# mattreturn1/ComputerVision_ObjectDetection_FeatureMatching

Measured on AMD Instinct MI355X. Metric: matches+homographies/sec (10k x 10k SIFT, 50k RANSAC iters) at 1/2/4/8 GPUs, higher is better.
Workload: dtype i8-MFMA exact-int distances (i32 acc), fp64 DLT/Jacobi, fp32 reprojection; 1 GPU; c4: one global batch of 256 scenes x 1 model set, 10000x10000 descriptors, maxIters 50000, scenes sharded over 1 GPU(s) (256 on rank 0); problems_per_gpu=256, global_batch=256, parallelism=dp1, batches_in_flight=16, dist_backend=nccl, hw_queues=24

## Files before the change

computervision_objectdetection_featurematching_amd/csrc/mim_internal.h:

```cpp
#pragma once
#include <hip/hip_runtime.h>
#include <stdint.h>

#include "knn_schedule.h"
#include "knn_topk_merge.h"

namespace mim {

constexpr int kDim = 128;
constexpr int kTileRows = 64;
constexpr int kTileBytes = kTileRows * kDim;
constexpr int kNormWords = 4 * kTileRows;
constexpr int kWave = 64;
#ifndef MIM_KNN_STAGE
#define MIM_KNN_STAGE 4
#endif
constexpr int kKnnStage = MIM_KNN_STAGE;

struct SetDev {
    const int8_t* frag;
    const int* norm;
    const float* f32;
    const float2* kp;
    int n;
    int n_tiles;
    int* flags;
};

struct PrepJob {
    const float* src;
    int8_t* frag;
    int* norm;
    int* flags;
    int n;
    int tile0;
};

struct Top2 {
    float k1; int i1; float k2; int i2;
};

struct ProbDev {
    SetDev q, t;
    int nsplit;
    int q_pad;
    long long part_off;
    long long good_off;
    long long it_off;
};


struct HamWork {
    const uint32_t* q;
    const uint32_t* t;
    Top2* out;
    int nq;
    int q0;
    int r0, r1;
    int wdw;
    int pad_;
};

struct HamCrossWork {
    HamWork w;
    uint32_t* colmin;
};

struct CrossDev {
    const uint32_t* colmin;
    int shadow;
    int pad_;
};


struct FltWork {
    const float* q;
    const float* t;
    Top2* out;
    int nq;
    int q0;
    int r0, r1;
    int dim;
    int dp;
};


struct TopkHamWork {
    const uint32_t* q;
    const uint32_t* t;
    TopkEnt* out;
    int nq;
    int q0;
    int r0, r1;
    int wdw;
    int pad_;
};

struct TopkFltWork {
    const float* q;
    const float* t;
    TopkEnt* out;
    int nq;
    int q0;
    int r0, r1;
    int dim;
    int dp;
    int nt;
    int vec;
};

struct TopkProb {
    const TopkEnt* parts;
    int32_t* idx;
    float* dist;
    int nq;
    int nsplit;
    int q_pad;
    int pad_;
};

struct RansacState {
    long long stream_pos;
    int produced;
    int fail_iter;
    int fail_run;
    int niters;
    int max_good;
    int best_iter;
    int next_iter;
    int done;
    int n;
    int active;
    int lo_max;
    unsigned long long modM;
    float sa, sb;
    float smax;
    int defer;
};

struct RansacParams {
    double thresh;
    double conf;
    int max_iters;
    float ratio;
    int min_good, min_inliers;
    double det_lo, det_hi;
    int cand_cap;
    int rep_cap;
};

}

namespace mim {
constexpr int kCandPerProblem = 1024;
constexpr int kIrrBlock = 16384;
constexpr int kRansacDefSlots = 16;
#ifndef MIM_CHECK_PER
#define MIM_CHECK_PER 4
#endif
constexpr int kRansacDefRoundAttempts = 256 * MIM_CHECK_PER;
constexpr int kIrrCap = 4096;

struct SamplerClass {
    long long base;
    int leader;
    int cwlen;
    int delta;
    int wlen;
    int pad_[2];
};
struct SamplerClassSlot {
    unsigned long long key;
    int end;
    int pad_;
};

struct RansacBufs {
    RansacState* state;
    int4* samples;
    float* hyp;
    int* counts;
    int2* bounds;
    double* best_h;
    int* cand;
    int* ncand;
    int* cex;
    double* cH;
    int* decided;
    uint8_t* flags;
    uint8_t* irr_bits;
    long long flag_cap;
    int* irr;
    int* irr_cnt;
    uint32_t* pass_bits;
    void* chains;
    int2* defer;
    int* defer_n;
    int def_rounds;
    int irr_blocks;
    SamplerClass* cls;
    SamplerClassSlot* cls_tab;
    int cls_tab_n;
    const uint32_t* stream;
    long long stream_len;
    float4* inl;
    uint4* tiles;
    int* err;
    hipStream_t s2;
    hipEvent_t ev_fork;
    hipEvent_t ev_samp[2];
};
}

#include <string>
#include <vector>
#include "../../include/mim.h"
namespace mim {
struct SiftWs;
SiftWs* sift_ws_create();
void sift_ws_destroy(SiftWs* w);
int sift_detect_compute(SiftWs* w, hipStream_t st, const uint8_t* img, int rows, int cols, long long step,
                        const uint8_t* mask, long long mstep, int max_kp, mim_keypoint* kps, float* desc, int* n_out,
                        std::string& err);
int sift_detect_compute_scales(std::vector<SiftWs*>& ws, hipStream_t st, const uint8_t* img, int rows, int cols,
                               long long step, int n_scales, const float* scales, int max_kp, mim_keypoint* kps,
                               float* desc, int* n_out, std::string& err);
int sift_resize_u8(SiftWs* w, hipStream_t st, const uint8_t* src, int rows, int cols, long long step, uint8_t* dst,
                   int drows, int dcols, double fx, double fy, std::string& err);
struct SiftDevOut {
    const mim_keypoint* kp;
    const float* desc;
    int n;
};
int sift_scales_device(std::vector<SiftWs*>& ws, hipStream_t st, const uint8_t* img, int rows, int cols,
                       long long step, int channels, int n_scales, const float* scales, SiftDevOut* out,
                       std::string& err);
int sift_bgr2gray_u8(SiftWs* w, hipStream_t st, const uint8_t* bgr, int rows, int cols, long long step, uint8_t* gray,
                     std::string& err);
int sift_copy_sets(const SiftDevOut* out, int n, float* const* ddesc, float2* const* dkp, hipStream_t st);
int sift_debug_pyramid(SiftWs* w, hipStream_t st, int* n_oct, int* orows, int* ocols, float* planes, long long cap,
                       long long* need, int* counters, std::string& err);
}
```

computervision_objectdetection_featurematching_amd/csrc/ransac.hip:

```cpp
#include <float.h>

#include <algorithm>
#include <climits>
#include <cstdio>
#include <cstdlib>
#include <vector>

#include "../../include/mim.h"
#include "mim_debug.h"
#include "mim_internal.h"

namespace mim {

__device__ __forceinline__ double d_hypot(double a, double b) {
    a = fabs(a);
    b = fabs(b);
    const bool ab = a > b;
    const double big = ab ? a : b, sm = ab ? b : a;
    const double r = sm / big;
    const double res = big * sqrt(1 + r * r);
    return (ab || b > 0) ? res : 0.0;
}

template <int n> __device__ __forceinline__ int pk(int i, int j) {
    static_assert(n <= 16, "packed index masks");
    return (int)(((unsigned)(i & 15) * (unsigned)((2 * n - 1 - i) & 31)) >> 1) + (j - i - 1);
}

template <int n> __device__ __forceinline__ int pk_any(int a, int b) {
    const int i = min(a, b), j = max(a, b);
    return pk<n>(i, j);
}

template <int n, int S>
__device__ void jacobi_fast(double* __restrict__ A, double* __restrict__ W, double* __restrict__ V,
                            double (&Ws)[n], int (&perm)[n]) {
#define AU(i, j) A[pk<n>((i), (j)) * S]
    const int trash = n * (n - 1) / 2 + n + n * n;
    const double eps = DBL_EPSILON;
#pragma unroll
    for (int i = 0; i < n; i++)
#pragma unroll
        for (int j = 0; j < n; j++) V[(i * n + j) * S] = i == j ? 1.0 : 0.0;
    int indR[n], indC[n];
#pragma unroll
    for (int k = 0; k < n; k++) {
        indR[k] = 0;
        indC[k] = 0;
        if (k < n - 1) {
            int m = k + 1;
            double mv = fabs(AU(k, k + 1));
#pragma unroll
            for (int i = k + 2; i < n; i++) {
                const double val = fabs(AU(k, i));
                if (mv < val) mv = val, m = i;
            }
            indR[k] = m;
        }
        if (k > 0) {
            int m = 0;
            double mv = fabs(AU(0, k));
#pragma unroll
            for (int i = 1; i < k; i++) {
                const double val = fabs(AU(i, k));
                if (mv < val) mv = val, m = i;
            }
            indC[k] = m;
        }
    }
    for (int iters = 0; iters < n * n * 30; iters++) {
        double vr[n], vc[n];
#pragma unroll
        for (int i = 0; i < n - 1; i++) vr[i] = A[(pk<n>(i, i + 1) + indR[i] - i - 1) * S];
#pragma unroll
        for (int i = 1; i < n; i++) vc[i] = A[pk_any<n>(indC[i], i) * S];
        int k = 0, l = indR[0];
        double mv = fabs(vr[0]), p = vr[0];
#pragma unroll
        for (int i = 1; i < n - 1; i++) {
            const double val = fabs(vr[i]);
            const bool u = mv < val;
            mv = u ? val : mv;
            k = u ? i : k;
            l = u ? indR[i] : l;
            p = u ? vr[i] : p;
        }
#pragma unroll
        for (int i = 1; i < n; i++) {
            const double val = fabs(vc[i]);
            const bool u = mv < val;
            mv = u ? val : mv;
            k = u ? indC[i] : k;
            l = u ? i : l;
            p = u ? vc[i] : p;
        }
        if (fabs(p) <= eps) break;
        const double wk = W[k * S], wl = W[l * S];
        double a0[n], b0[n], vk[n], vl[n];
#pragma unroll
        for (int i = 0; i < n; i++) {
            const bool vi = i != k && i != l;
            a0[i] = A[(vi ? pk_any<n>(i, k) : 0) * S];
            b0[i] = A[(vi ? pk_any<n>(i, l) : 0) * S];
            vk[i] = V[(k * n + i) * S];
            vl[i] = V[(l * n + i) * S];
        }
        const double y = (wl - wk) * 0.5;
        double t = fabs(y) + d_hypot(p, y);
        const double q = fabs(p) / t;
        double s = t * sqrt(1 + q * q);
        const double c = t / s;
        s = p / s;
        t = copysign(q, p) * p;
        s = y < 0 ? -s : s;
        t = y < 0 ? -t : t;
        AU(k, l) = 0;
        W[k * S] = wk - t;
        W[l * S] = wl + t;
        double rk[n], rl[n];
#pragma unroll
        for (int i = 0; i < n; i++) {
            const bool vi = i != k && i != l;
            const double na = a0[i] * c - b0[i] * s;
            const double nb = a0[i] * s + b0[i] * c;
            A[(vi ? pk_any<n>(i, k) : trash) * S] = na;
            A[(vi ? pk_any<n>(i, l) : trash) * S] = nb;
            rk[i] = vi ? na : 0.0;
            rl[i] = vi ? nb : 0.0;
            V[(k * n + i) * S] = vk[i] * c - vl[i] * s;
            V[(l * n + i) * S] = vk[i] * s + vl[i] * c;
        }
        int rkR = -1, rkC = -1, rlR = -1, rlC = -1;
        double bkR = 0, bkC = 0, blR = 0, blC = 0;
#pragma unroll
        for (int m = 0; m < n; m++) {
            const double ak = fabs(rk[m]), al = fabs(rl[m]);
            const bool u1 = m > k && (rkR < 0 || bkR < ak);
            const bool u2 = m < k && (rkC < 0 || bkC < ak);
            const bool u3 = m > l && (rlR < 0 || blR < al);
            const bool u4 = m < l && (rlC < 0 || blC < al);
            bkR = u1 ? ak : bkR; rkR = u1 ? m : rkR;
            bkC = u2 ? ak : bkC; rkC = u2 ? m : rkC;
            blR = u3 ? al : blR; rlR = u3 ? m : rlR;
            blC = u4 ? al : blC; rlC = u4 ? m : rlC;
        }
#pragma unroll
        for (int i = 0; i < n; i++) {
            indR[i] = (i == k && i < n - 1) ? rkR : ((i == l && i < n - 1) ? rlR : indR[i]);
            indC[i] = (i == k && i > 0) ? rkC : ((i == l && i > 0) ? rlC : indC[i]);
        }
    }
#pragma unroll
    for (int i = 0; i < n; i++) {
        Ws[i] = W[i * S];
        perm[i] = i;
    }
#pragma unroll
    for (int k = 0; k < n - 1; k++) {
// ... 953 lines not shown
        if (w < wave) r = max(r, wred[w]);
        all = max(all, wred[w]);
    }
    return r;
}

__device__ __forceinline__ int block_min(int v, int* wred) {
    const int lane = threadIdx.x & 63, wave = threadIdx.x >> 6, nw = blockDim.x >> 6;
    v = wave_min(v);
    __syncthreads();
    if (lane == 0) wred[wave] = v;
    __syncthreads();
    int r = INT_MAX;
    for (int w = 0; w < nw; ++w) r = min(r, wred[w]);
    return r;
}

__global__ __launch_bounds__(kWalkThreads) void ransac_walk_kernel(const RansacState* __restrict__ st,
                                                                    const uint8_t* __restrict__ flags, int wcap,
                                                                    int c1, const int* __restrict__ irr,
                                                                    const int* __restrict__ irr_cnt, int irr_blocks,
                                                                    ChainSegs* __restrict__ chains,
                                                                    const SamplerClass* __restrict__ cls) {
    __shared__ ChainWalkShared sh;
    const int p = blockIdx.x, tid = threadIdx.x, lane = tid & 63;
    const SamplerClass C = cls[p];
    ChainSegs* G = chains + p;
    if (C.leader < 0) {
        if (tid == 0) G->T = -1;
        return;
    }
    const int wlen = C.delta + C.wlen;
    const int pl = C.leader;
    const uint8_t* F = flags + (long long)pl * wcap;
    const int nb = min((wlen + kIrrBlock - 1) / kIrrBlock, kIrrBlocksMax);
    {
        const int cnt = tid < nb ? irr_cnt[(long long)pl * irr_blocks + tid] : 0;
        const int bad = tid < nb && cnt < 0 ? tid : INT_MAX;
        int total;
        const int off = block_excl_sum(max(cnt, 0), sh.wred, total);
        const int cut = min(block_min(bad, sh.wred2), nb);
        if (tid <= nb) sh.boff[tid] = tid < nb ? off : 0;
        __syncthreads();
        if (tid == 0) {
            sh.cut = cut;
            sh.n_entries = cut > 0 ? sh.boff[cut - 1] + irr_cnt[(long long)pl * irr_blocks + cut - 1] : 0;
            sh.limit = min(wlen, cut * kIrrBlock);
            sh.stop = 0;
        }
        __syncthreads();
    }
    int s = C.delta, nwalk = 0, limit = sh.limit;
    const int E = sh.n_entries, cut = sh.cut;
    for (int eb = 0; eb < E; eb += kChainEntries) {
        const int ee = min(E, eb + kChainEntries);
        for (int e = eb + tid; e < ee; e += kWalkThreads) {
            int lo = 0, hi = cut - 1;
            while (lo < hi) {
                const int mid = (lo + hi + 1) >> 1;
                if (sh.boff[mid] <= e) lo = mid; else hi = mid - 1;
            }
            const int q = irr[((long long)pl * irr_blocks + lo) * kIrrCap + (e - sh.boff[lo])];
            sh.q[e - eb] = q;
            sh.f[e - eb] = F[q];
        }
        __syncthreads();
        if (tid < 64) {
            bool stop = false;
            for (int e0 = eb; e0 < ee && !stop; e0 += 64) {
                const int e = e0 + lane;
                const int q = e < ee ? sh.q[e - eb] : INT_MAX;
                const int f = e < ee ? (int)sh.f[e - eb] : 0;
                for (;;) {
                    const unsigned long long m = __ballot(q >= s && q < limit && ((q - s) & 3) == 0);
                    if (!m) break;
                    const int k = uni(__builtin_ctzll(m));
                    const int qq = __builtin_amdgcn_readlane(q, k), ff = __builtin_amdgcn_readlane(f, k);
                    if (ff == kAttemptSerial || nwalk == kChainSegs) {
                        limit = qq;
                        stop = true;
                        break;
                    }
                    if (lane == 0) {
                        G->seg_s[nwalk] = s;
                        G->seg_q[nwalk] = qq;
                        G->seg_f[nwalk] = (uint8_t)ff;
                    }
                    ++nwalk;
                    s = uni(qq + 4 + ((ff & 0x7F) >> 1));
                }
            }
            if (lane == 0 && stop) sh.stop = 1;
        }
        __syncthreads();
        if (sh.stop) break;
    }
    if (tid < 64) {
        if (lane == 0) {
            const int tail = s < limit ? (limit - s + 3) >> 2 : 0;
            G->seg_s[nwalk] = s;
            sh.nseg = nwalk;
            sh.tail = tail;
            G->nseg = nwalk;
            G->tail = tail;
            G->s_end = s + 4 * tail;
            G->wbase = C.base;
            G->wlen = wlen;
        }
    }
    __syncthreads();
    const int nseg = sh.nseg;
    int v[kWalkSegsPer], sum = 0;
#pragma unroll
    for (int k = 0; k < kWalkSegsPer; ++k) {
        const int j = kWalkSegsPer * tid + k;
        v[k] = j < nseg ? ((G->seg_q[j] - G->seg_s[j]) >> 2) + 1 : (j == nseg ? sh.tail : 0);
        sum += v[k];
    }
    int total;
    int base = block_excl_sum(sum, sh.wred, total);
#pragma unroll
    for (int k = 0; k < kWalkSegsPer; ++k) {
        const int j = kWalkSegsPer * tid + k;
        if (j <= nseg + 1) G->A[j] = base;
        if (j <= nseg)
            for (int b = (base + kCheckBlock - 1) / kCheckBlock; b * kCheckBlock < base + v[k] && b < kChainBlk; ++b)
                G->blk_seg[b] = j;
        base += v[k];
    }
    if (tid == 0) G->T = total;
}

__device__ __forceinline__ int chain_pos(const ChainSegs* G, int j, int t, bool& irregular) {
    irregular = j < G->nseg && t == G->A[j + 1] - 1;
    return irregular ? G->seg_q[j] : G->seg_s[j] + 4 * (t - G->A[j]);
}

__device__ __forceinline__ int chain_seg(const ChainSegs* G, int t) {
    int lo = 0, hi = G->nseg;
    while (lo < hi) {
        const int mid = (lo + hi + 1) >> 1;
        if (G->A[mid] <= t) lo = mid; else hi = mid - 1;
    }
    return lo;
}


constexpr int kCheckPer = MIM_CHECK_PER;
constexpr int kCheckSegs = 8;
#ifndef MIM_PROBE_CHECK
#define MIM_PROBE_CHECK 0
#endif
constexpr int kDefSlots = kRansacDefSlots;
#ifndef MIM_CHECK_LDS
#define MIM_CHECK_LDS 0
#endif
constexpr int kCheckLdsPts = MIM_CHECK_LDS ? 2048 : 1;
static_assert(kCheckBlock * kCheckPer == kRansacDefRoundAttempts, "check round size shared with api.cpp");

__device__ __attribute__((noinline)) bool check_deferred(int qe, const uint32_t* __restrict__ stream, long long slen,
                                                         unsigned N, unsigned long long modM,
                                                         const float4* __restrict__ P) {
    const long long qq = qe < 0 ? -(long long)qe - 1 : qe;
    int ix[4];
    if (qe < 0) {
        resolve_at(qq, stream, slen, N, modM, ix);
    } else {
#pragma unroll
        for (int k = 0; k < 4; ++k) ix[k] = (int)fastmod(stream[qq + k], modM, N);
    }
    const float4 a = P[ix[0]], bp = P[ix[1]], c = P[ix[2]], d = P[ix[3]];
    const float s4[8] = {a.x, a.y, bp.x, bp.y, c.x, c.y, d.x, d.y};
    const float t4[8] = {a.z, a.w, bp.z, bp.w, c.z, c.w, d.z, d.w};
    return check_subset(s4, t4);
}

#ifndef MIM_CHECK_OCC
#define MIM_CHECK_OCC 1
#endif
__global__ __launch_bounds__(kCheckBlock, MIM_CHECK_OCC) void ransac_check_kernel(const ChainSegs* __restrict__ chains,
                                                                   const ProbDev* __restrict__ probs,
                                                                   const float4* __restrict__ pts,
                                                                   const RansacState* __restrict__ st,
                                                                   const uint32_t* __restrict__ stream, long long slen,
                                                                   uint32_t* __restrict__ pass_bits, int wcap, int bpp,
                                                                   int2* __restrict__ defer, int* __restrict__ defer_n,
                                                                   int def_rounds, int n_probs) {
    __shared__ uint32_t words[kCheckBlock * kCheckPer / 32];
    __shared__ int def_t[kCheckBlock * kCheckPer], def_q[kCheckBlock * kCheckPer];
    __shared__ int4 seg_tab[kCheckSegs];
    __shared__ int n_def;
    __shared__ float4 spts[kCheckLdsPts];
    const int x = blockIdx.x & 7, jx = blockIdx.x >> 3, np8 = (n_probs + 7) >> 3;
    const int p = x + 8 * (jx % np8), kb0 = jx / np8, lane = threadIdx.x & 63;
    if (p >= n_probs) return;
    const ChainSegs* G = chains + p;
    const int T = G->T;
    if (T <= 0) return;
    const RansacState S = st[p];
    const float4* P = pts + probs[p].good_off;
    const bool lds = MIM_CHECK_LDS && S.n <= kCheckLdsPts;
    if (lds) {
        for (int i = threadIdx.x; i < S.n; i += kCheckBlock) spts[i] = P[i];
    }
    for (int b = kb0; b * kCheckBlock * kCheckPer < T; b += bpp) {
    const int base = b * kCheckBlock * kCheckPer;
    const int nseg = G->nseg;
    const int bb = base / kCheckBlock;
    const int j0 = bb < kChainBlk ? G->blk_seg[bb] : chain_seg(G, base);
    if (threadIdx.x < kCheckSegs) {
        const int j = j0 + threadIdx.x;
        seg_tab[threadIdx.x] = make_int4(G->A[min(j, nseg + 1)], G->A[min(j + 1, nseg + 1)], G->seg_s[min(j, nseg)],
                                         G->seg_q[min(j, max(nseg - 1, 0))]);
    }
    int segA[kCheckSegs];
#pragma unroll
    for (int k = 1; k < kCheckSegs; ++k) segA[k] = j0 + k <= nseg ? G->A[j0 + k] : INT_MAX;
    const unsigned N = (unsigned)S.n;
    if (threadIdx.x == 0) n_def = 0;
    __syncthreads();
    int q[kCheckPer];
    bool irr[kCheckPer], valid[kCheckPer];
#pragma unroll
    for (int r = 0; r < kCheckPer; ++r) {
        const int t = base + r * kCheckBlock + threadIdx.x;
        valid[r] = t < T;
        int k = 0;
#pragma unroll
        for (int i = 1; i < kCheckSegs; ++i) k += t >= segA[i];
        const int4 e = seg_tab[k];
        int j = j0 + k, pos;
        bool irregular;
        if (j < nseg && t >= e.y) {
            while (j < nseg && t >= G->A[j + 1]) ++j;
            pos = chain_pos(G, j, t, irregular);
        } else {
            irregular = j < nseg && t == e.y - 1;
            pos = irregular ? e.w : e.z + 4 * (t - e.x);
        }
        q[r] = valid[r] ? (int)(G->wbase + pos) : 0;
        irr[r] = valid[r] && irregular;
    }
    typedef unsigned uint4a4 __attribute__((ext_vector_type(4), aligned(4)));
    unsigned raw[kCheckPer][4];
#pragma unroll
    for (int r = 0; r < kCheckPer; ++r) {
        const uint4a4 v = *reinterpret_cast<const uint4a4*>(stream + q[r]);
        raw[r][0] = v.x; raw[r][1] = v.y; raw[r][2] = v.z; raw[r][3] = v.w;
    }
    int idx[kCheckPer][4];
#pragma unroll
    for (int r = 0; r < kCheckPer; ++r)
#pragma unroll
        for (int k = 0; k < 4; ++k) idx[r][k] = valid[r] ? (int)fastmod(raw[r][k], S.modM, N) : 0;
    float4 g[kCheckPer][4];
    __syncthreads();
    if (lds) {
#pragma unroll
        for (int r = 0; r < kCheckPer; ++r)
#pragma unroll
            for (int k = 0; k < 4; ++k) g[r][k] = spts[idx[r][k]];
    } else {
#pragma unroll
        for (int r = 0; r < kCheckPer; ++r)
#pragma unroll
            for (int k = 0; k < 4; ++k) g[r][k] = P[idx[r][k]];
    }
    const bool listed = b < def_rounds;
#pragma unroll
    for (int r = 0; r < kCheckPer; ++r) {
        const float s4[8] = {g[r][0].x, g[r][0].y, g[r][1].x, g[r][1].y, g[r][2].x, g[r][2].y, g[r][3].x, g[r][3].y};
        const float t4[8] = {g[r][0].z, g[r][0].w, g[r][1].z, g[r][1].w, g[r][2].z, g[r][2].w, g[r][3].z, g[r][3].w};
        bool clear = true;
        const bool pass32 = MIM_PROBE_CHECK == 3 ? (s4[0] + s4[1] + s4[2] + s4[3] + s4[4] + s4[5] + s4[6] + s4[7] +
                                                    t4[0] + t4[1] + t4[2] + t4[3] + t4[4] + t4[5] + t4[6] + t4[7]) > 4000.f
                          : MIM_PROBE_CHECK == 2 ? s4[0] != t4[1] : check_subset_fp32(s4, t4, clear);
        MIM_DEBUG_CHECK(!valid[r] || !clear || pass32 == check_subset(s4, t4),
                        "[check] fp32 checkSubset %d differs from fp64 (p=%d t=%d)\n", (int)pass32, p,
                        base + r * kCheckBlock + (int)threadIdx.x);
        const bool defer = MIM_PROBE_CHECK == 0 && valid[r] && (irr[r] || !clear);
        const unsigned long long m = __ballot(valid[r] && !defer && pass32);
        const int wl = (r * kCheckBlock + (threadIdx.x & ~63)) >> 5;
        if (lane == 0) words[wl] = (uint32_t)m;
        if (lane == 32) words[wl + 1] = (uint32_t)(m >> 32);
        if (defer) {
            const int slot = atomicAdd(&n_def, 1);
            def_t[slot] = r * kCheckBlock + threadIdx.x;
            def_q[slot] = irr[r] ? -q[r] - 1 : q[r];
        }
    }
    __syncthreads();
    MIM_DEBUG_PRINT(threadIdx.x == 0 && (p == 0 || p == 100), "[check] p=%d b=%d bpp=%d T=%d nseg=%d n_def=%d wlen=%d\n",
                    p, b, bpp, T, nseg, n_def, G->wlen);
    const int nl = listed ? min(n_def, kDefSlots) : 0;
    if (listed && threadIdx.x == 0) defer_n[(long long)p * def_rounds + b] = nl;
    if (threadIdx.x < nl)
        defer[((long long)p * def_rounds + b) * kDefSlots + threadIdx.x] =
            make_int2(base + def_t[threadIdx.x], def_q[threadIdx.x]);
    if (n_def > nl) {
        for (int e = nl + threadIdx.x; e < n_def; e += kCheckBlock) {
            const int tl = def_t[e];
            if (check_deferred(def_q[e], stream, slen, N, S.modM, P)) atomicOr(&words[tl >> 5], 1u << (tl & 31));
        }
        __syncthreads();
    }
    uint32_t* PB = pass_bits + (long long)p * (wcap / 32);
    if (threadIdx.x < kCheckBlock * kCheckPer / 32 && (base + 32 * (int)threadIdx.x) < T)
        PB[(base >> 5) + threadIdx.x] = words[threadIdx.x];
    __syncthreads();
    }
}

__global__ __launch_bounds__(256) void ransac_check_defer_kernel(const ChainSegs* __restrict__ chains,
                                                                 const ProbDev* __restrict__ probs,
                                                                 const float4* __restrict__ pts,
                                                                 const RansacState* __restrict__ st,
                                                                 const uint32_t* __restrict__ stream, long long slen,
                                                                 uint32_t* __restrict__ pass_bits, int wcap,
                                                                 const int2* __restrict__ defer,
                                                                 const int* __restrict__ defer_n, int def_rounds,
                                                                 int nblk, int n_probs) {
    const int p = blockIdx.x / nblk;
    const int j = (blockIdx.x % nblk) * 256 + threadIdx.x, round = j / kDefSlots, e = j % kDefSlots;
    if (p >= n_probs || round >= def_rounds) return;
    const int T = chains[p].T;
    if (round * (kCheckBlock * kCheckPer) >= T) return;
    const long long rr = (long long)p * def_rounds + round;
    if (e >= defer_n[rr]) return;
    const int2 en = defer[rr * kDefSlots + e];
    const int t = en.x, qe = en.y;
    if (check_deferred(qe, stream, slen, (unsigned)st[p].n, st[p].modM, pts + probs[p].good_off))
        atomicOr(pass_bits + (long long)p * (wcap / 32) + (t >> 5), 1u << (t & 31));
}

template <class Fn>
__device__ __forceinline__ void pass_visit(const uint32_t* __restrict__ PB, int t0, int t1, Fn&& fn) {
    if (t0 >= t1) return;
    const int wl = (t1 - 1) >> 5;
    for (int w0 = t0 >> 5; w0 <= wl; w0 += 8) {
        uint32_t wd[8];
#pragma unroll
        for (int k = 0; k < 8; ++k) wd[k] = PB[min(w0 + k, wl)];
#pragma unroll
        for (int k = 0; k < 8; ++k) {
            const int w = w0 + k;
            if (w > wl) break;
            const int lo_b = max(t0 - 32 * w, 0), hi_b = min(t1 - 32 * w, 32);
            const uint32_t rm = (hi_b == 32 ? 0xFFFFFFFFu : ((1u << hi_b) - 1)) & ~((1u << lo_b) - 1);
            uint32_t bits = wd[k] & rm;
            while (bits) {
                const int bit = __builtin_ctz(bits);
                bits &= bits - 1;
                fn(32 * w + bit);
            }
        }
    }
}

struct ChainCountShared {
    int wred[kChainThreads / 64];
    int wred2[kChainThreads / 64];
    int t_need;
};

__global__ __launch_bounds__(kChainThreads) void ransac_count_kernel(RansacState* __restrict__ st,
                                                                     const ProbDev* __restrict__ probs,
                                                                     const ChainSegs* __restrict__ chains,
                                                                     const uint32_t* __restrict__ pass_bits,
                                                                     const uint8_t* __restrict__ flags, int wcap,
                                                                     int4* __restrict__ samples, int c1,
                                                                     const SamplerClass* __restrict__ cls) {
    __shared__ ChainCountShared sh;
    const int p = blockIdx.x, tid = threadIdx.x;
    const ChainSegs* G = chains + p;
    const int T = G->T;
    if (T < 0) return;
    RansacState S = st[p];
    const int target = min(c1, S.niters);
    if (S.produced >= target) return;
    const long long wbase = G->wbase;
    const uint32_t* PB = pass_bits + (long long)p * (wcap / 32);
    const int words = (T + 31) >> 5;
    const int wpt = (words + kChainThreads - 1) / kChainThreads;
    const int t0 = min(T, tid * wpt * 32), t1 = min(T, t0 + wpt * 32);
    int cnt = 0, first = -1, last = -1;
    pass_visit(PB, t0, t1, [&](int t) {
        if (first < 0) first = t;
        last = t;
        ++cnt;
    });
    int total;
    const int base = block_excl_sum(cnt, sh.wred, total);
    const int v0 = -1 - S.fail_run;
    int last_all;
    const int prev = block_excl_max(cnt ? last : INT_MIN, v0, sh.wred2, last_all);
    int ev = (cnt && first - prev - 1 >= 10000) ? prev + 10000 : kNoEvent;
    if (tid == 0 && T - 1 - last_all >= 10000) ev = min(ev, last_all + 10000);
    const int t_fail = block_min(ev, sh.wred);
    const int need = target - S.produced;
    if (tid == 0) sh.t_need = kNoEvent;
    __syncthreads();
    if (base < need && need <= base + cnt) {
        int k = need - base;
        pass_visit(PB, t0, t1, [&](int t) {
            if (--k == 0) sh.t_need = t;
        });
    }
    __syncthreads();
    const int t_need = sh.t_need;
    int keep;
    if (t_fail < t_need) {
        int before = 0;
        if (cnt && last < t_fail) before = cnt;
        else if (cnt && first < t_fail) pass_visit(PB, t0, t1, [&](int t) { before += t < t_fail; });
        int tot_before;
        block_excl_sum(before, sh.wred, tot_before);
        keep = tot_before;
    } else {
        keep = t_need != kNoEvent ? need : total;
    }
    if (base < keep) {
        int4* out = samples + probs[p].it_off + S.produced;
        int r = base, j = -1, a_next = 0, a_j = 0, s_j = 0, q_j = 0;
        pass_visit(PB, t0, t1, [&](int t) {
            if (r < keep) {
                if (j < 0 || t >= a_next) {
                    j = j < 0 ? chain_seg(G, t) : j + 1;
                    while (j < G->nseg && t >= G->A[j + 1]) ++j;
                    a_j = G->A[j];
                    a_next = G->A[j + 1];
                    s_j = G->seg_s[j];
                    q_j = j < G->nseg ? G->seg_q[j] : 0;
                }
                const bool irregular = j < G->nseg && t == a_next - 1;
                const int pos = irregular ? q_j : s_j + 4 * (t - a_j);
                out[r] = make_int4((int)(wbase + pos), irregular ? -2 : -1, 0, 0);
            }
            ++r;
        });
    }
    if (tid == 0) {
        if (t_fail < t_need) {
            S.produced += keep;
            S.fail_iter = S.produced;
            S.fail_run = 10000;
        } else if (t_need != kNoEvent) {
            const int j = chain_seg(G, t_need);
            bool irregular;
            const int pos = chain_pos(G, j, t_need, irregular);
            const int len = irregular ? 4 + ((flags[(long long)cls[p].leader * wcap + pos] & 0x7F) >> 1) : 4;
            S.produced = target;
            S.stream_pos = wbase + pos + len;
            S.fail_run = 0;
        } else {
            S.produced += total;
            S.fail_run = total > 0 ? T - 1 - last_all : S.fail_run + T;
            S.stream_pos = wbase + G->s_end;
        }
        store_sampler_state(st + p, S);
    }
}


// ... 1872 lines not shown
                            for (int j = 0; j < 8; ++j) s += sh.A[8 * i + j] * sh.d[j];
                            temp_d[i] = -s + 2 * sh.v[i];
                        }
                        double dS = 0;
                        for (int i = 0; i < 8; ++i) dS += sh.d[i] * temp_d[i];
                        const double R = (Scur - Sd) / (fabs(dS) > DBL_EPSILON ? dS : 1);
                        if (R > Rhi) {
                            lambda *= 0.5;
                            if (lambda < lc) lambda = 0;
                        } else if (R < Rlo) {
                            double t = 0;
                            for (int i = 0; i < 8; ++i) t += sh.d[i] * sh.v[i];
                            double nu = (Sd - Scur) / (fabs(t) > DBL_EPSILON ? t : 1) + 2;
                            nu = fmin(fmax(nu, 2.), 10.);
                            if (lambda == 0) {
                                const double maxval = inv_diag_max8(ew, eperm, sh.J9 + 36);
                                lambda = lc = 1. / maxval;
                                nu *= 0.5;
                            }
                            lambda *= nu;
                        }
                        if (tid == 0) {
                            sh.lambda = lambda;
                            sh.lc = lc;
                            sh.accept = Sd < Scur;
                            if (sh.accept) {
                                sh.S = Sd;
                                for (int i = 0; i < 8; ++i) sh.x[i] = sh.xd[i];
                            }
                        }
                    }
                    wsync();
                    if (sh.accept) {
#if MIM_LM_MERGE
                        rinf = rinf_d;
#else
                        for (int i = 0; i < 8; ++i) x[i] = sh.x[i];
                        lm_normal(X, k, x, sh.lm, sh.nrm, rinf);
#endif
                        if (tid == 0) {
                            int e = 0;
                            for (int a = 0; a < 8; ++a)
                                for (int b = a; b < 8; ++b, ++e) sh.A[a * 8 + b] = sh.A[b * 8 + a] = sh.nrm[e];
                            for (int i = 0; i < 8; ++i) sh.v[i] = sh.nrm[36 + i];
                            sh.rinf = rinf;
                        }
                    }
                    MIM_RT_MARK(t_norm);
                    ++iter;
                    if (tid == 0) sh.proceed = iter < 10 && sh.dinf >= FLT_EPSILON && sh.rinf >= FLT_EPSILON;
                    wsync();
                    const bool proceed = sh.proceed;
                    wsync();
                    if (!proceed) break;
                }
#if MIM_REFINE_TIMING
                rt_iters = iter;
#endif
                if (tid < 8) sh.H[tid] = sh.x[tid];
                wsync();
            } else if (tid == 0) {
                for (int i = 0; i < 9; ++i) sh.H[i] = sh.Hb[i];
            }
            wsync();
        } else {
            for (int i = tid; i < ng; i += 64) mask[i] = 0;
            if (tid == 0) sh.n_inl = 0;
        }
    }
    wsync();
    if (tid != 0) return;
#if MIM_REFINE_TIMING
    {
        const unsigned long long tot = wall_clock64() - rt_start;
        if (tot > 20000)
            printf("[refine-timing] p=%d ng=%d inl=%d iters=%d total=%llu mask=%llu refit=%llu norm0=%llu "
                   "solve=%llu cost=%llu norm=%llu (us x100) niters=%d produced=%d done=%d small=%d\n", p, ng,
                   sh.n_inl, rt_iters, tot, t_mask, t_refit, t_norm0, t_solve, t_cost, t_norm, S.niters, S.produced,
                   S.done, (int)(S.n < kSmallMaxN));
    }
#endif
    res.n_inl = ok ? sh.n_inl : 0;
    if (!ok) {
        res.status = (S.active && S.fail_iter == -2) ? MIM_STREAM_SHORT : MIM_EMPTY_H;
    } else {
        for (int i = 0; i < 9; ++i) res.H[i] = sh.H[i];
        const double* H = sh.H;
        double t = H[0] * (H[4] * H[8] - H[5] * H[7]);
        t -= H[1] * (H[3] * H[8] - H[5] * H[6]);
        t += H[2] * (H[3] * H[7] - H[4] * H[6]);
        res.det = t;
        if (raw) res.status = MIM_ACCEPTED;
        else if (res.n_inl < prm.min_inliers) res.status = MIM_FEW_INLIERS;
        else {
            const double ad = fabs(t);
            res.status = (ad < prm.det_lo || ad > prm.det_hi) ? MIM_BAD_DET : MIM_ACCEPTED;
        }
    }
    results[p] = res;
}

size_t ransac_chain_bytes() { return sizeof(ChainSegs); }

__global__ __launch_bounds__(256) void rng_stream_kernel(const unsigned long long* __restrict__ seg_state,
                                                         uint32_t* __restrict__ out, long long len, int seg,
                                                         int n_seg) {
    const int i = blockIdx.x * blockDim.x + threadIdx.x;
    if (i >= n_seg) return;
    unsigned long long st = seg_state[i];
    const long long p0 = (long long)i * seg;
    const int m = (int)min((long long)seg, len - p0);
    for (int k = 0; k < m; ++k) {
        out[p0 + k] = (uint32_t)st;
        st = (unsigned long long)(uint32_t)st * 4164903690ull + (st >> 32);
    }
}

void launch_rng_stream(const unsigned long long* seg_state, uint32_t* out, long long len, int seg, int n_seg,
                       hipStream_t s) {
    rng_stream_kernel<<<(n_seg + 255) / 256, 256, 0, s>>>(seg_state, out, len, seg, n_seg);
}

void ransac_enqueue(const RansacParams& prm, int n_probs, const ProbDev* probs, const float4* pts,
                    const int* n_good, const RansacBufs& b, uint8_t* masks, mim_result* results, int raw,
                    hipStream_t s, void (*mark)(void*, const char*, hipStream_t), void* mark_ctx, int exact_all) {
    if (n_probs <= 0) return;
    ransac_init_kernel<<<(n_probs + 255) / 256, 256, 0, s>>>(b.state, n_good, n_probs, prm.max_iters, prm.min_good,
                                                             b.best_h);
    const int max_iters = prm.max_iters > 1 ? prm.max_iters : 1;
    const char* sw = getenv("MIM_SAMPLER_WALK");
    const int use_chain = !(sw && sw[0] == '1');
    int first = max_iters <= 4096 ? 512 : 4096;
    if (const char* fc = getenv("MIM_FIRST_CHUNK")) first = std::max(1, atoi(fc));
    int c0 = 0, chunk = first;
    const float thr2 = (float)(prm.thresh * prm.thresh);
    if (!exact_all) ransac_tiles_kernel<<<n_probs, 256, 0, s>>>(b.state, probs, pts, b.tiles);
    const bool split = b.s2 && !exact_all;
    hipStream_t ss = split ? b.s2 : s;
    if (split) {
        (void)hipEventRecord(b.ev_fork, s);
        (void)hipStreamWaitEvent(ss, b.ev_fork, 0);
        mark(mark_ctx, "fork", ss);
    }
    int ci = 0, c1_first = 0;
    const int cap = prm.cand_cap > 0 ? std::min(prm.cand_cap, kCandCap) : kCandCap;
    const char* pe = getenv("MIM_PRESCREEN");
    const int prescreen = (pe && pe[0] == '0') ? 0 : 1;
    const char* se = getenv("MIM_SETTLE");
    const int settle = (se && se[0] == '0') ? 0 : 1;
    const char* we = getenv("MIM_WINNER_H");
    const int winner_h = !we ? 2 : we[0] == '1' ? 1 : we[0] == '0' ? 0 : 2;
    int min_blocks = kSamplerMinBlocks;
    if (const char* mb = getenv("MIM_SAMPLER_MIN_BLOCKS")) min_blocks = std::max(0, atoi(mb));
    const char* she = getenv("MIM_SAMPLER_SHARE");
    const int share = (she && she[0] == '0') ? 0 : 1;
    const char* spe = getenv("MIM_SHARE_SPREAD");
    while (c0 < max_iters) {
        const int c1 = (int)std::min<long long>((long long)c0 + chunk, max_iters);
        const int wcap = (int)(std::min<long long>((long long)(c1 - c0) * 28 + 4096, b.flag_cap / std::max(n_probs, 1)) & ~63LL);
        const int west = (int)std::min<long long>(wcap, (long long)(c1 - c0) * kAttemptRateEst + 4096);
        const int bppw_cap = std::max(1, wcap / kAttemptSpan);
        const int bppw = (std::max((west + kAttemptSpan - 1) / kAttemptSpan,
                                   std::min(bppw_cap, (min_blocks + n_probs - 1) / n_probs)) + 7) / 8 * 8;
        const int rep_cap = prm.rep_cap > 0 ? std::min(prm.rep_cap, kAttemptRepCap) : kAttemptRepCap;
        const int spread = std::min(spe ? std::max(0, atoi(spe)) : wcap / 16, wcap / 2);
        const bool dbg_ncls = getenv("MIM_DEBUG_NCLASS") != nullptr;
        if (dbg_ncls && split) (void)hipStreamSynchronize(s);
        ransac_class_kernel<<<1, kClassThreads, 0, ss>>>(b.state, n_probs, c1, wcap, share, spread, b.cls_tab,
                                                         b.cls_tab_n, b.cls);
        if (dbg_ncls) {
            std::vector<SamplerClass> hc(n_probs);
            (void)hipMemcpyAsync(hc.data(), b.cls, sizeof(SamplerClass) * n_probs, hipMemcpyDeviceToHost, ss);
            (void)hipStreamSynchronize(ss);
            int nw = 0, nc = 0;
            for (int i = 0; i < n_probs; ++i) {
                nw += hc[i].leader >= 0;
                nc += hc[i].leader == i;
            }
            fprintf(stderr, "[mim] sampler chunk [%d,%d): windowed %d classes %d\n", c0, c1, nw, nc);
        }
        ransac_attempt_kernel<<<n_probs * bppw, 256, 0, ss>>>(b.state, b.stream, b.stream_len, b.flags, b.irr_bits, wcap,
                                                             bppw, c1, rep_cap, n_probs, b.cls);
        mark(mark_ctx, "attempt", ss);
        if (use_chain) {
            ChainSegs* chains = reinterpret_cast<ChainSegs*>(b.chains);
            const int bpp_irr = (west + kIrrBlock - 1) / kIrrBlock;
            ransac_irr_kernel<<<n_probs * bpp_irr, 256, 0, ss>>>(b.state, b.irr_bits, wcap, bpp_irr, c1, b.irr,
                                                               b.irr_cnt, b.irr_blocks, b.cls);
            ransac_walk_kernel<<<n_probs, kWalkThreads, 0, ss>>>(b.state, b.flags, wcap, c1, b.irr, b.irr_cnt,
                                                                 b.irr_blocks, chains, b.cls);
            mark(mark_ctx, "chain", ss);
            constexpr int kChkSpan = kCheckBlock * kCheckPer;
            const int bpp_chk = std::max((west / 4 + kChkSpan) / kChkSpan,
                                         std::min(std::max(1, wcap / 4 / kChkSpan), (min_blocks + n_probs - 1) / n_probs));
            ransac_check_kernel<<<8 * ((n_probs + 7) / 8) * bpp_chk, kCheckBlock, 0, ss>>>(
                chains, probs, pts, b.state, b.stream, b.stream_len, b.pass_bits, wcap, bpp_chk, b.defer, b.defer_n,
                b.def_rounds, n_probs);
            if (b.def_rounds > 0) {
                const int nblk = (b.def_rounds * kDefSlots + 255) / 256;
                ransac_check_defer_kernel<<<n_probs * nblk, 256, 0, ss>>>(chains, probs, pts, b.state, b.stream,
                                                                        b.stream_len, b.pass_bits, wcap, b.defer,
                                                                        b.defer_n, b.def_rounds, nblk, n_probs);
            }
            mark(mark_ctx, "check", ss);
            ransac_count_kernel<<<n_probs, kChainThreads, 0, ss>>>(b.state, probs, chains, b.pass_bits, b.flags, wcap,
                                                                  b.samples, c1, b.cls);
            mark(mark_ctx, "chain", ss);
        }
        ransac_small_kernel<<<n_probs, kSmallThreads, 0, ss>>>(b.state, probs, pts, b.stream, b.stream_len, b.samples,
                                                              c1, b.err);
        ransac_sample_kernel<<<n_probs, 64, 0, ss>>>(b.state, probs, pts, b.stream, b.stream_len, b.samples, c1, b.err,
                                                    b.flags, b.irr_bits, wcap, b.cls);
        mark(mark_ctx, "sample", ss);
        if (split) {
            (void)hipEventRecord(b.ev_samp[ci & 1], ss);
            (void)hipStreamWaitEvent(s, b.ev_samp[ci & 1], 0);
            mark(mark_ctx, "join", s);
        }
        ++ci;
        const int bpp256 = (c1 - c0 + 255) / 256;
        const int bppb = (c1 - c0 + kBoundThreads - 1) / kBoundThreads;
        if (exact_all) {
            const int bpp64 = (c1 - c0 + 63) / 64;
            ransac_hypo_kernel<<<n_probs * bpp64, 64, 0, s>>>(b.state, probs, pts, b.samples, b.stream, b.hyp, b.counts, c0, c1,
                                                             bpp64);
            mark(mark_ctx, "hypo", s);
            ransac_score_kernel<<<n_probs * bpp256, 256, 0, s>>>(b.state, probs, pts, b.hyp, b.counts, c0, c1,
                                                                bpp256, thr2);
            mark(mark_ctx, "score", s);
            ransac_select_kernel<<<n_probs, 64, 0, s>>>(b.state, probs, b.counts, c1, prm.conf);
            mark(mark_ctx, "select", s);
            if (getenv("MIM_DEBUG_TRACE") && n_probs == 1) {
                std::vector<int> hc(c1 - c0);
                std::vector<int4> hs(c1 - c0);
                (void)hipMemcpyAsync(hc.data(), b.counts + c0, sizeof(int) * (c1 - c0), hipMemcpyDeviceToHost, s);
                (void)hipMemcpyAsync(hs.data(), b.samples + c0, sizeof(int4) * (c1 - c0), hipMemcpyDeviceToHost, s);
                (void)hipStreamSynchronize(s);
                for (int i = 0; i < c1 - c0; ++i)
                    fprintf(stderr, "[trace] %d %d %d %d %d %d\n", c0 + i, hc[i], hs[i].x, hs[i].y, hs[i].z, hs[i].w);
            }
        } else {
            if (c0 == 0)
                ransac_bound_mfma_kernel<true><<<8 * ((n_probs + 7) / 8) * bppb, kBoundThreads, 0, s>>>(
                    b.state, probs, pts, b.samples, b.stream, b.tiles, b.bounds, c0, c1, bppb, thr2, n_probs);
            else
                ransac_bound_mfma_kernel<false><<<8 * ((n_probs + 7) / 8) * bppb, kBoundThreads, 0, s>>>(
                    b.state, probs, pts, b.samples, b.stream, b.tiles, b.bounds, c0, c1, bppb, thr2, n_probs);
            mark(mark_ctx, "score", s);
            if (getenv("MIM_CHECK_BOUNDS")) {
                unsigned long long* dst = nullptr;
                unsigned long long h[6] = {0, 0, 0, 0, 0, 0};
                if (hipMalloc(&dst, sizeof h) == hipSuccess) {
                    (void)hipMemsetAsync(dst, 0, sizeof h, s);
                    const int bpp64 = (c1 - c0 + 63) / 64;
                    ransac_bound_check_kernel<<<n_probs * bpp64, 64, 0, s>>>(b.state, probs, pts, b.samples, b.stream,
                                                                             b.bounds, c0, c1, bpp64, thr2, dst);
                    (void)hipMemcpyAsync(h, dst, sizeof h, hipMemcpyDeviceToHost, s);
                    (void)hipStreamSynchronize(s);
                    (void)hipFree(dst);
                }
                fprintf(stderr, "[mim] bound check chunk [%d,%d): checked %llu lo_viol %llu hi_viol %llu valid_mismatch %llu "
                        "mean_width %.2f tight %llu\n", c0, c1, h[0], h[1], h[2], h[3], h[0] ? (double)h[4] / h[0] : 0.0, h[5]);
            }
            const int L = c0 == 0 ? 0 : 1;
            ransac_cand_kernel<<<n_probs, kCandThreads, 0, s>>>(b.state, probs, b.bounds, c1, b.cand, b.ncand, L,
                                                                cap);
            if (prescreen) {
                ransac_prescreen_kernel<<<n_probs * kPreWaves, 64, 0, s>>>(b.state, probs, b.bounds, pts, b.samples,
                                                                          b.stream, b.cand, b.ncand, b.cex, b.cH,
                                                                          b.decided, thr2, L, cap);
                if (settle)
                    ransac_settle_kernel<<<n_probs, 64, 0, s>>>(b.state, probs, b.bounds, b.cand, b.ncand, b.cex, b.cH,
                                                                b.decided, L, cap, winner_h);
            }
            mark(mark_ctx, "cand", s);
            if (prescreen && getenv("MIM_CHECK_PRESCREEN")) {
                unsigned long long* dst = nullptr;
                unsigned long long h[2] = {0, 0};
                if (hipMalloc(&dst, sizeof h) == hipSuccess) {
                    (void)hipMemsetAsync(dst, 0, sizeof h, s);
                    ransac_prescreen_check_kernel<<<n_probs * (kCandCap / 64), 64, 0, s>>>(
                        b.state, probs, pts, b.samples, b.stream, b.cand, b.ncand, b.cex, b.decided, b.bounds,
                        thr2, L, cap, dst);
                    (void)hipMemcpyAsync(h, dst, sizeof h, hipMemcpyDeviceToHost, s);
                    (void)hipStreamSynchronize(s);
                    (void)hipFree(dst);
                }
                fprintf(stderr, "[mim] prescreen check chunk [%d,%d): decided %llu mismatch %llu\n", c0, c1, h[0], h[1]);
            }
            if (getenv("MIM_DEBUG_NCAND")) {
                std::vector<int> h(2 * n_probs), dec((size_t)2 * n_probs * kCandCap);
                (void)hipMemcpyAsync(h.data(), b.ncand, sizeof(int) * 2 * n_probs, hipMemcpyDeviceToHost, s);
                if (prescreen)
                    (void)hipMemcpyAsync(dec.data(), b.decided, sizeof(int) * dec.size(), hipMemcpyDeviceToHost, s);
                (void)hipStreamSynchronize(s);
                long long sum = 0, sum2 = 0; int mx = 0;
                for (int i = 0; i < n_probs; ++i) {
                    const int nl = std::min(h[2 * i + L], cap);
                    sum += h[2 * i + L];
                    mx = std::max(mx, h[2 * i + L]);
                    for (int k = 0; k < nl; ++k) sum2 += prescreen ? dec[(size_t)(2 * i + L) * kCandCap + k] == 0 : 1;
                }
                fprintf(stderr, "[mim] chunk [%d,%d): candidates mean %.1f max %d undecided mean %.1f\n", c0, c1,
                        (double)sum / n_probs, mx, (double)sum2 / n_probs);
            }
            ransac_exact_kernel<<<n_probs * kExactWaves * (L + 1), 64, 0, s>>>(b.state, probs, pts, b.samples, b.stream,
                                                                             b.cand, b.ncand, b.bounds, b.cex, b.cH,
                                                                             thr2, L, cap, b.decided, prescreen);
            mark(mark_ctx, "exact", s);
            ransac_replay_kernel<<<n_probs, 64, 0, s>>>(b.state, probs, pts, b.samples, b.stream, b.bounds, b.cand,
                                                        b.ncand, b.cex, b.cH, c1, prm.conf, thr2, b.best_h, L,
                                                        c1_first, cap);
            mark(mark_ctx, "select", s);
        }
        if (c0 == 0) c1_first = c1;
        c0 = c1;
        chunk = 1 << 30;
    }
    if (getenv("MIM_CHECK_BESTH")) {
        std::vector<double> bh((size_t)n_probs * 9);
        std::vector<RansacState> hs(n_probs);
        (void)hipMemcpyAsync(bh.data(), b.best_h, sizeof(double) * bh.size(), hipMemcpyDeviceToHost, s);
        (void)hipMemcpyAsync(hs.data(), b.state, sizeof(RansacState) * n_probs, hipMemcpyDeviceToHost, s);
        (void)hipStreamSynchronize(s);
        int with = 0, without = 0;
        for (int i = 0; i < n_probs; ++i)
            if (hs[i].active && hs[i].best_iter >= 0 && hs[i].n >= kSmallMaxN) (bh[9 * i + 8] != 0.0 ? with : without)++;
        fprintf(stderr, "[mim] best_h: %d problems with the exact pass's fp64 bestModel, %d without\n", with, without);
    }
    ransac_refine_kernel<<<(n_probs + kRW - 1) / kRW, kRT, 0, s>>>(b.state, probs, pts, n_good, b.samples, b.stream, b.inl,
                                                                  masks, results, prm, raw, b.best_h, exact_all, n_probs);
    mark(mark_ctx, "refine", s);
}

}
```

Measured before the change: 37130 problems/s.

## Enable LDS point staging in RANSAC check kernel and cap blocks per problem

Turns on LDS staging of the point set in the RANSAC check kernel by default. The points are prefetched into registers before the first round and written to shared memory after the index computation, so the global load latency overlaps other work. It also shrinks the deferred-attempt index array to uint16 and makes blocks return early when their first round is past the chain length. The check grid now targets a fixed blocks-per-problem count (default 16) instead of scaling with the estimated attempt count, so each block loops over more rounds and the staging cost is spread across them. The trade-off is fewer blocks, which can leave the GPU under-occupied, plus extra register and LDS pressure from the 2048-entry staging buffer.

```diff
diff --git a/computervision_objectdetection_featurematching_amd/csrc/check_grid.h b/computervision_objectdetection_featurematching_amd/csrc/check_grid.h
--- /dev/null
+++ b/computervision_objectdetection_featurematching_amd/csrc/check_grid.h
@@ -0,0 +1,31 @@
+#pragma once
+#include <algorithm>
+
+namespace mim {
+
+#ifndef MIM_CHECK_PER
+#define MIM_CHECK_PER 4
+#endif
+constexpr int kRansacDefRoundAttempts = 256 * MIM_CHECK_PER;
+#ifndef MIM_CHECK_BPP
+#define MIM_CHECK_BPP 16
+#endif
+constexpr int kCheckBpp = MIM_CHECK_BPP;
+
+struct CheckGrid {
+    int bpp;
+    int rounds;
+};
+
+inline CheckGrid check_grid(int n_probs, int west, int wcap, int min_blocks, int target = kCheckBpp) {
+    constexpr int span = kRansacDefRoundAttempts;
+    n_probs = std::max(n_probs, 1);
+    const int est = std::max(west, 0) / 4 / span + 1;
+    const int cap = std::max(1, std::max(wcap, 0) / 4 / span);
+    const int floor_bpp = std::min(cap, (std::max(min_blocks, 0) + n_probs - 1) / n_probs);
+    const int bpp = (std::max(std::min(std::max(target, 1), est), floor_bpp) + 7) / 8 * 8;
+    const int max_rounds = (std::max(wcap, 0) / 4 + span - 1) / span;
+    return {bpp, std::max(1, (max_rounds + bpp - 1) / bpp)};
+}
+
+}
diff --git a/computervision_objectdetection_featurematching_amd/csrc/mim_internal.h b/computervision_objectdetection_featurematching_amd/csrc/mim_internal.h
--- a/computervision_objectdetection_featurematching_amd/csrc/mim_internal.h
+++ b/computervision_objectdetection_featurematching_amd/csrc/mim_internal.h
@@ -2,6 +2,7 @@
 #include <hip/hip_runtime.h>
 #include <stdint.h>
 
+#include "check_grid.h"
 #include "knn_schedule.h"
 #include "knn_topk_merge.h"
 
@@ -155,10 +156,6 @@
 constexpr int kCandPerProblem = 1024;
 constexpr int kIrrBlock = 16384;
 constexpr int kRansacDefSlots = 16;
-#ifndef MIM_CHECK_PER
-#define MIM_CHECK_PER 4
-#endif
-constexpr int kRansacDefRoundAttempts = 256 * MIM_CHECK_PER;
 constexpr int kIrrCap = 4096;
 
 struct SamplerClass {
diff --git a/computervision_objectdetection_featurematching_amd/csrc/ransac.hip b/computervision_objectdetection_featurematching_amd/csrc/ransac.hip
--- a/computervision_objectdetection_featurematching_amd/csrc/ransac.hip
+++ b/computervision_objectdetection_featurematching_amd/csrc/ransac.hip
@@ -4,6 +4,7 @@
 #include <climits>
 #include <cstdio>
 #include <cstdlib>
+#include <type_traits>
 #include <vector>
 
 #include "../../include/mim.h"
@@ -1263,10 +1264,8 @@
 #define MIM_PROBE_CHECK 0
 #endif
 constexpr int kDefSlots = kRansacDefSlots;
-#ifndef MIM_CHECK_LDS
-#define MIM_CHECK_LDS 0
-#endif
-constexpr int kCheckLdsPts = MIM_CHECK_LDS ? 2048 : 1;
+constexpr int kCheckLdsPts = 2048;
+constexpr int kCheckStagePer = kCheckLdsPts / kCheckBlock;
 static_assert(kCheckBlock * kCheckPer == kRansacDefRoundAttempts, "check round size shared with api.cpp");
 
 __device__ __attribute__((noinline)) bool check_deferred(int qe, const uint32_t* __restrict__ stream, long long slen,
@@ -1298,23 +1297,30 @@
                                                                    int2* __restrict__ defer, int* __restrict__ defer_n,
                                                                    int def_rounds, int n_probs) {
     __shared__ uint32_t words[kCheckBlock * kCheckPer / 32];
-    __shared__ int def_t[kCheckBlock * kCheckPer], def_q[kCheckBlock * kCheckPer];
+    __shared__ uint16_t def_t[kCheckBlock * kCheckPer];
+    __shared__ int def_q[kCheckBlock * kCheckPer];
     __shared__ int4 seg_tab[kCheckSegs];
     __shared__ int n_def;
     __shared__ float4 spts[kCheckLdsPts];
+    static_assert(kCheckBlock * kCheckPer <= 65536, "def_t holds an attempt's index in its round");
     const int x = blockIdx.x & 7, jx = blockIdx.x >> 3, np8 = (n_probs + 7) >> 3;
     const int p = x + 8 * (jx % np8), kb0 = jx / np8, lane = threadIdx.x & 63;
     if (p >= n_probs) return;
     const ChainSegs* G = chains + p;
     const int T = G->T;
-    if (T <= 0) return;
+    if (kb0 * (kCheckBlock * kCheckPer) >= T) return;
     const RansacState S = st[p];
     const float4* P = pts + probs[p].good_off;
-    const bool lds = MIM_CHECK_LDS && S.n <= kCheckLdsPts;
+    const bool lds = S.n <= kCheckLdsPts;
+    float4 stg[kCheckStagePer];
     if (lds) {
-        for (int i = threadIdx.x; i < S.n; i += kCheckBlock) spts[i] = P[i];
-    }
-    for (int b = kb0; b * kCheckBlock * kCheckPer < T; b += bpp) {
+#pragma unroll
+        for (int k = 0; k < kCheckStagePer; ++k) {
+            const int i = k * kCheckBlock + threadIdx.x;
+            stg[k] = i < S.n ? P[i] : make_float4(0.f, 0.f, 0.f, 0.f);
+        }
+    }
+    auto round = [&](const int b, auto first) __attribute__((always_inline)) {
     const int base = b * kCheckBlock * kCheckPer;
     const int nseg = G->nseg;
     const int bb = base / kCheckBlock;
@@ -1365,6 +1371,13 @@
 #pragma unroll
         for (int k = 0; k < 4; ++k) idx[r][k] = valid[r] ? (int)fastmod(raw[r][k], S.modM, N) : 0;
     float4 g[kCheckPer][4];
+    if (decltype(first)::value && lds) {
+#pragma unroll
+        for (int k = 0; k < kCheckStagePer; ++k) {
+            const int i = k * kCheckBlock + threadIdx.x;
+            if (i < S.n) spts[i] = stg[k];
+        }
+    }
     __syncthreads();
     if (lds) {
 #pragma unroll
@@ -1383,9 +1396,10 @@
         const float s4[8] = {g[r][0].x, g[r][0].y, g[r][1].x, g[r][1].y, g[r][2].x, g[r][2].y, g[r][3].x, g[r][3].y};
         const float t4[8] = {g[r][0].z, g[r][0].w, g[r][1].z, g[r][1].w, g[r][2].z, g[r][2].w, g[r][3].z, g[r][3].w};
         bool clear = true;
-        const bool pass32 = MIM_PROBE_CHECK == 3 ? (s4[0] + s4[1] + s4[2] + s4[3] + s4[4] + s4[5] + s4[6] + s4[7] +
-                                                    t4[0] + t4[1] + t4[2] + t4[3] + t4[4] + t4[5] + t4[6] + t4[7]) > 4000.f
-                          : MIM_PROBE_CHECK == 2 ? s4[0] != t4[1] : check_subset_fp32(s4, t4, clear);
+        const bool fifth = raw[r][0] * 0x9E3779B1u < 0x33333333u;
+        const bool pass32 = MIM_PROBE_CHECK == 3 ? fifth && (s4[0] + s4[1] + s4[2] + s4[3] + s4[4] + s4[5] + s4[6] + s4[7] +
+                                                            t4[0] + t4[1] + t4[2] + t4[3] + t4[4] + t4[5] + t4[6] + t4[7]) > -4e30f
+                          : MIM_PROBE_CHECK == 2 ? fifth && s4[0] != t4[1] + 4e30f : check_subset_fp32(s4, t4, clear);
         MIM_DEBUG_CHECK(!valid[r] || !clear || pass32 == check_subset(s4, t4),
                         "[check] fp32 checkSubset %d differs from fp64 (p=%d t=%d)\n", (int)pass32, p,
                         base + r * kCheckBlock + (int)threadIdx.x);
@@ -1396,7 +1410,7 @@
         if (lane == 32) words[wl + 1] = (uint32_t)(m >> 32);
         if (defer) {
             const int slot = atomicAdd(&n_def, 1);
-            def_t[slot] = r * kCheckBlock + threadIdx.x;
+            def_t[slot] = (uint16_t)(r * kCheckBlock + threadIdx.x);
             def_q[slot] = irr[r] ? -q[r] - 1 : q[r];
         }
     }
@@ -1419,7 +1433,9 @@
     if (threadIdx.x < kCheckBlock * kCheckPer / 32 && (base + 32 * (int)threadIdx.x) < T)
         PB[(base >> 5) + threadIdx.x] = words[threadIdx.x];
     __syncthreads();
-    }
+    };
+    round(kb0, std::true_type{});
+    for (int b = kb0 + bpp; b * (kCheckBlock * kCheckPer) < T; b += bpp) round(b, std::false_type{});
 }
 
 __global__ __launch_bounds__(256) void ransac_check_defer_kernel(const ChainSegs* __restrict__ chains,
@@ -3598,6 +3614,11 @@
     const int winner_h = !we ? 2 : we[0] == '1' ? 1 : we[0] == '0' ? 0 : 2;
     int min_blocks = kSamplerMinBlocks;
     if (const char* mb = getenv("MIM_SAMPLER_MIN_BLOCKS")) min_blocks = std::max(0, atoi(mb));
+    int chk_bpp = kCheckBpp, chk_min_blocks = min_blocks;
+    if (const char* cb = getenv("MIM_CHECK_BPP")) {
+        chk_bpp = std::max(1, atoi(cb));
+        chk_min_blocks = 0;
+    }
     const char* she = getenv("MIM_SAMPLER_SHARE");
     const int share = (she && she[0] == '0') ? 0 : 1;
     const char* spe = getenv("MIM_SHARE_SPREAD");
@@ -3636,9 +3657,7 @@
             ransac_walk_kernel<<<n_probs, kWalkThreads, 0, ss>>>(b.state, b.flags, wcap, c1, b.irr, b.irr_cnt,
                                                                  b.irr_blocks, chains, b.cls);
             mark(mark_ctx, "chain", ss);
-            constexpr int kChkSpan = kCheckBlock * kCheckPer;
-            const int bpp_chk = std::max((west / 4 + kChkSpan) / kChkSpan,
-                                         std::min(std::max(1, wcap / 4 / kChkSpan), (min_blocks + n_probs - 1) / n_probs));
+            const int bpp_chk = check_grid(n_probs, west, wcap, chk_min_blocks, chk_bpp).bpp;
             ransac_check_kernel<<<8 * ((n_probs + 7) / 8) * bpp_chk, kCheckBlock, 0, ss>>>(
                 chains, probs, pts, b.state, b.stream, b.stream_len, b.pass_bits, wcap, bpp_chk, b.defer, b.defer_n,
                 b.def_rounds, n_probs);
```

Result: no change. 37430 problems/s, median of 3 (+0.8%).
